# Newiz430/CellSegmentation

Measured on AMD Instinct MI355X. Metric: tiles/sec fwd+bwd (ResNet-50 MIL, 299x299), higher is better.
Workload: dtype bf16; 1 GPU; ResNet-50 tile classifier (train_tile.py --scratch semantics: fwd + CE + full bwd + Adam), bag=64 tiles of 299x299x3 per GPU, freeze_bn=True; tiles_per_gpu=64, parallelism=dp1

## Files before the change

cellsegmentation_amd/_lib.py:

```python
import ctypes
import os
from ctypes import POINTER, Structure, c_char_p, c_double, c_float, c_int, c_int32, c_int64, c_longlong, c_size_t, c_void_p

_HERE = os.path.dirname(os.path.abspath(__file__))
FLAVOUR = os.environ.get("CELLSEG_LIB_FLAVOUR", "")
if FLAVOUR not in ("", "ab"):
    raise RuntimeError(f"CELLSEG_LIB_FLAVOUR={FLAVOUR!r}: expected unset or 'ab'")
LIB_PATH = os.path.join(_HERE, f"libcellseg_hip_{FLAVOUR}.so" if FLAVOUR else "libcellseg_hip.so")

CS_F32, CS_BF16 = 0, 1
CS_ACT_NONE, CS_ACT_RELU, CS_ACT_SILU, CS_ACT_SIGMOID = 0, 1, 2, 3
CS_BN_BWD_OWN_RELU, CS_BN_BWD_FROZEN = 0x100, 0x200


class CsConvGeom(Structure):
    _fields_ = [(n, c_int32) for n in ("N", "H", "W", "C", "K", "R", "S", "stride", "pad", "P", "Q", "groups")]


class CsStageDesc(Structure):
    _fields_ = ([(n, c_void_p) for n in ("w", "gamma", "beta", "mean", "var", "conv_bias", "w_khwc", "w_chwk", "scale", "shift", "rstd")]
                + [("eps", c_float)] + [(n, c_int32) for n in ("K", "Cin", "R", "S", "Cp", "Kp", "block0", "fwd_packed", "bwd_packed")])


class CellsegLibraryMissing(RuntimeError):
# ... 50 lines not shown
    "cs_sgd_step_dev": (c_int, [_P, _P, c_int, c_int, _P, c_int, _P, c_double, c_double, c_int, c_int, _P]),
    "cs_sample_sum_workspace": (c_size_t, [c_int, c_int, c_int]),
    "cs_sample_sum": (c_int, [_P, _P, c_int, c_float, _P, _P, c_int, c_int, c_int, _P]),
    "cs_maxpool3x3s2_fwd": (c_int, [_P, c_int, _P, _P, c_int, c_int, c_int, c_int, c_int, c_int, _P]),
    "cs_maxpool3x3s2_bwd": (c_int, [_P, _P, _P, c_int, _P, c_int, c_int, c_int, c_int, c_int, c_int, _P]),
    "cs_gap_avgmax_fwd": (c_int, [_P, c_int, _P, _P, c_int, c_int, c_int, c_int, _P]),
    "cs_gap_avgmax_bwd": (c_int, [_P, _P, _P, c_int, _P, c_int, c_int, c_int, c_int, c_int, _P]),
    "cs_linear_fwd": (c_int, [_P, _P, _P, _P, _P, c_int, c_int, c_int, c_int, _P]),
    "cs_linear_bwd_workspace": (c_size_t, [c_int, c_int, c_int]),
    "cs_linear_bwd": (c_int, [_P, _P, _P, _P, c_int, _P, _P, _P, c_int, c_int, c_int, c_int, _P, _P]),
    "cs_loss_words": (c_int, []),
    "cs_softmax_ce": (c_int, [_P, _P, c_float, _P, _P, c_int, c_int, _P]),
    "cs_softmax_prob1": (c_int, [_P, _P, c_int, c_int, _P]),
    "cs_softmax_argmax": (c_int, [_P, _P, c_int, c_int, _P]),
    "cs_mse": (c_int, [_P, _P, c_int, c_int, _P, _P, c_int, _P]),
    "cs_bn_accum_words": (c_size_t, [c_int]),
    "cs_bn_accum_read": (c_int, [_P, c_int, _P, _P]),
    "cs_bn_stats": (c_int, [_P, c_int, c_longlong, c_int, _P, _P, _P]),
    "cs_bn_partial_workspace": (c_size_t, [c_longlong, c_int]),
    "cs_bn_finalize": (c_int, [_P, c_longlong, c_float, c_float, _P, _P, _P, _P, c_int, _P]),
    "cs_bn_apply": (c_int, [_P, c_int, _P, _P, _P, _P, _P, c_int, _P, c_longlong, c_int, _P]),
    "cs_bn_apply_stats": (c_int, [_P, c_int, _P, c_float, c_float, _P, _P, _P, _P, _P, c_int, _P, _P, _P, c_longlong, c_int, _P]),
    "cs_bn_bwd_reduce": (c_int, [_P, _P, c_int, _P, _P, _P, _P, c_int, c_longlong, c_int, _P, _P, _P]),
    "cs_bn_bwd_apply": (c_int, [_P, _P, c_int, _P, _P, _P, _P, c_int, _P, c_longlong, c_int, _P, _P, _P, _P]),
    "cs_dwconv_fwd": (c_int, [POINTER(CsConvGeom), c_int, _P, _P, _P, _P, c_int, _P, _P]),
    "cs_dwconv_fwd_stats_workspace": (c_size_t, [POINTER(CsConvGeom)]),
    "cs_dwconv_fwd_stats": (c_int, [POINTER(CsConvGeom), c_int, _P, _P, _P, _P, POINTER(c_int), _P]),
    "cs_bn_partial_fold": (c_int, [_P, c_int, c_int, _P, _P]),
    "cs_dwconv_dgrad": (c_int, [POINTER(CsConvGeom), c_int, _P, _P, _P, _P]),
    "cs_dwconv_wgrad": (c_int, [POINTER(CsConvGeom), c_int, _P, _P, _P, _P, _P]),
    "cs_dwconv_wgrad_oihw": (c_int, [POINTER(CsConvGeom), c_int, _P, _P, _P, _P, _P]),
    "cs_dw_weights_hwc_multi": (c_int, [_P, c_int, ctypes.c_longlong, _P]),
    "cs_dwconv_wgrad_workspace": (ctypes.c_size_t, [POINTER(CsConvGeom)]),
    "cs_se_scale": (c_int, [_P, c_int, _P, _P, c_int, c_int, c_int, _P]),
    "cs_se_scale_bwd_dx": (c_int, [_P, c_int, _P, _P, _P, c_int, c_int, c_int, _P]),
    "cs_rowscale_add": (c_int, [_P, c_int, _P, _P, _P, c_int, c_longlong, _P]),
    "cs_bilinear_ac_fwd": (c_int, [_P, c_int, _P, c_int, c_int, c_int, c_int, c_int, c_int, _P]),
    "cs_bilinear_ac_bwd": (c_int, [_P, _P, c_int, _P, c_int, c_int, c_int, c_int, c_int, c_int, _P]),
    "cs_concat_channels": (c_int, [_P, _P, c_int, _P, c_longlong, c_int, c_int, _P]),
    "cs_split_channels": (c_int, [_P, c_int, _P, _P, c_longlong, c_int, c_int, _P]),
    "cs_tile_gather": (c_int, [_P, c_int, c_int, c_int, _P, _P, c_longlong, c_int, POINTER(c_float), POINTER(c_float), c_int, _P, _P]),
    "cs_stage_augmented_workspace": (c_size_t, [c_longlong]),
    "cs_stage_augmented": (c_int, [_P, c_int, c_int, c_int, _P, _P, _P, _P, _P, c_int, c_longlong, c_int, c_int, POINTER(c_float),
                                   POINTER(c_float), c_int, _P, _P, c_size_t, _P]),
    "cs_dice_fwd": (c_int, [_P, _P, c_int, c_longlong, c_float, c_int, _P, _P, _P]),
    "cs_dice_bwd": (c_int, [_P, _P, _P, c_int, c_longlong, c_float, c_int, _P, _P]),
    "cs_softmax_channel_fwd": (c_int, [_P, _P, c_int, c_int, c_longlong, c_int, _P]),
    "cs_softmax_channel_bwd": (c_int, [_P, _P, _P, c_int, c_int, c_longlong, c_int, _P]),
    "cs_segmented_topk_workspace": (c_size_t, [c_longlong]),
    "cs_segmented_topk": (c_int, [_P, _P, _P, _P, c_int, c_int, c_longlong, _P, _P, _P, c_size_t, _P]),
    "cs_stem_pair_input": (c_int, [_P, c_int, c_int, c_int, c_int, _P, _P]),
    "cs_stem_pair_from_nchw": (c_int, [_P, c_int, c_int, c_int, c_int, _P, _P]),
    "cs_stem_fwd_packed": (c_int, [c_int, c_int, c_int, c_int, _P, _P, _P, c_int, _P, _P, _P]),
    "cs_stem_pair_weights": (c_int, [_P, c_int, c_int, _P, _P]),
    "cs_stem_fwd": (c_int, [c_int, c_int, c_int, c_int, c_int, _P, _P, _P, _P, c_int, _P, _P, _P, _P]),
    "cs_stem_wgrad_splits": (c_int, [c_int, c_int, c_int, c_int]),
    "cs_stem_wgrad": (c_int, [c_int, c_int, c_int, c_int, c_int, _P, _P, _P, c_int, _P]),
    "cs_stem_unpair_slabs": (c_int, [_P, c_int, c_int, _P, _P]),
    "cs_segmented_order": (c_int, [_P, _P, c_int, c_int, c_longlong, _P, _P]),
    "cs_threshold_select": (c_int, [_P, _P, c_longlong, c_float, _P, _P, _P, c_size_t, _P]),
    "cs_evaluate_tile_counts": (c_int, [_P, _P, _P, _P, c_float, c_longlong, _P, _P]),
    "cs_paint_tile_masks": (c_int, [_P, c_longlong, _P, _P, c_int, c_int, c_int, _P, _P]),
    "cs_prune_excess": (c_int, [_P, c_longlong, c_int, c_longlong, _P, _P, _P]),
    "cs_detect_quantize": (c_int, [_P, c_longlong, _P, _P]),
    "cs_detect_blur": (c_int, [_P, c_int, c_int, c_int, c_int, _P, c_int, _P, c_int, _P, _P]),
    "cs_stitch_workspace": (c_size_t, [c_int, c_int]),
    "cs_stitch_patches": (c_int, [_P, c_int, c_int, c_int, _P, c_int, c_int, _P, _P, c_size_t, _P]),
    "cs_stitch_logits": (c_int, [_P, c_int, c_int, c_int, c_int, c_int, _P, c_int, c_int, _P, _P]),
    "cs_detect_grid_size": (c_int, [c_int, c_int, c_int, c_int]),
    "cs_detect_meanshift": (c_int, [_P, c_int, c_int, c_int, c_int, c_int, c_double, c_int, _P, _P, _P]),
    "cs_detect_cluster_workspace": (c_size_t, [c_int, c_int]),
    "cs_detect_cluster": (c_int, [_P, _P, c_int, c_int, c_double, _P, c_int, c_int, c_int, _P, _P, _P, _P, c_size_t, _P]),
    "cs_detect_edt_workspace": (c_size_t, [c_int, c_int, c_int, c_int]),
    "cs_detect_edt_sq": (c_int, [_P, c_int, c_int, c_int, c_int, c_int, _P, _P, c_size_t, _P]),
    "cs_detect_edt_smooth": (c_int, [_P, c_int, c_int, c_int, c_int, c_int, _P, _P, c_size_t, _P]),
    "cs_morph_max_site_width": (c_int, []),
    "cs_morph_workspace": (c_size_t, [c_int, c_int, c_int]),
    "cs_morph_nearest": (c_int, [_P, c_int, c_int, c_int, c_int, c_int, _P, _P, _P, c_size_t, _P]),
    "cs_morph_binary": (c_int, [_P, c_int, c_int, c_int, c_int, c_int, c_int, _P, _P, c_size_t, _P]),
    "cs_morph_expand_labels": (c_int, [_P, c_int, c_int, c_int, c_int, _P, _P, c_size_t, _P]),
    "cs_regions_workspace": (c_size_t, [c_int, c_int, c_int]),
    "cs_regions_label": (c_int, [_P, c_int, c_int, c_int, c_int, _P, _P, c_size_t, _P]),
    "cs_regions_areas": (c_int, [_P, c_int, c_int, c_int, c_int, _P, _P, c_size_t, _P]),
    "cs_regions_filter": (c_int, [_P, c_int, c_int, c_int, c_int, c_int, c_int, _P, _P, c_size_t, _P]),
    "cs_regions_remove_small": (c_int, [_P, c_int, c_int, c_int, c_int, c_int, c_int, _P, _P, c_size_t, _P]),
    "cs_regions_threshold": (c_int, [_P, c_longlong, c_float, _P, _P]),
    "cs_regions_hsv_gate": (c_int, [_P, _P, c_longlong, c_int, _P, _P]),
    "cs_regions_number": (c_int, [_P, c_int, c_int, c_int, c_int, _P, _P, c_size_t, _P]),
    "cs_regions_measure": (c_int, [_P, _P, c_int, c_int, c_int, c_int, c_int, c_int, _P, _P, _P, _P, _P, _P, _P, c_size_t, _P]),
    "cs_regions_split_workspace": (c_size_t, [c_int, c_int, c_int, c_int]),
    "cs_regions_split": (c_int, [_P, c_int, c_int, c_int, c_int, _P, _P, _P, c_int, _P, _P, _P, _P, c_size_t, _P]),
    "cs_regions_geodesic_workspace": (c_size_t, [c_int, c_int, c_int, c_int]),
    "cs_regions_split_geodesic": (c_int, [_P, c_int, c_int, c_int, c_int, _P, _P, _P, c_int, c_int, c_int, _P, _P, _P, _P, _P, _P, c_size_t, _P]),
    "cs_regions_measure_labels": (c_int, [_P, _P, c_int, c_int, c_int, c_int, _P, _P, _P, _P, _P, _P, _P]),
    "cs_regions_edges_labels": (c_int, [_P, c_int, c_int, c_int, _P, _P]),
    "cs_regions_shape_labels": (c_int, [_P, _P, c_int, c_int, c_int, c_int, _P, _P, _P, _P]),
    "cs_regions_hull_max_side": (c_int, []),
    "cs_regions_hull_labels": (c_int, [_P, c_int, c_int, c_int, c_int, _P, _P, _P]),
    "cs_regions_match_workspace": (c_size_t, [c_int, c_int, c_int]),
    "cs_regions_match_labels": (c_int, [_P, _P, c_int, c_int, c_int, c_int, c_int, _P, _P, _P, _P, _P, _P, _P, _P, c_size_t, _P]),
    "cs_regions_overlap_workspace": (c_size_t, [c_int, c_int, c_int, c_int]),
    "cs_regions_overlap_labels": (c_int, [_P, _P] + [c_int] * 6 + [_P] * 13 + [c_size_t, _P]),
    "cs_regions_hausdorff_stage_runs": (c_int, []),
    "cs_regions_hausdorff_workspace": (c_size_t, [c_int, c_int, c_int]),
    "cs_regions_hausdorff_labels": (c_int, [_P, _P] + [c_int] * 5 + [_P] * 7 + [c_size_t, _P]),
    "cs_score_workspace": (c_size_t, [c_int, c_longlong]),
# ... 47 lines not shown
```

cellsegmentation_amd/engine.py:

```python
from collections import namedtuple
from types import SimpleNamespace

import torch

from . import _capture
from . import kernels as K

ACT_NONE, ACT_RELU, ACT_SILU = K.CS_ACT_NONE, K.CS_ACT_RELU, K.CS_ACT_SILU

PACKED = True
PACKED_TRAIN_BN = True


class ConvUnit:
    kind = "conv"

    def __init__(self, name, conv, bn, act, src, dst, res=None):
        self.name, self.conv, self.bn, self.act = name, conv, bn, act
        self.src, self.dst, self.res = src, dst, res
        self.grouped = conv.groups != 1
        if self.grouped:
            cg = conv.in_channels // conv.groups
            if conv.in_channels != conv.out_channels or conv.in_channels % 64 != 0 or 64 % cg != 0 or conv.bias is not None:
                raise NotImplementedError(f"{name}: grouped convolution needs C == K, C % 64 == 0, (C/groups) | 64, no bias "
                                          "(the ResNeXt 32x4d / 32x8d 3x3 layers)")
        self._cache = None

    def params(self):
        out = [("weight", self.conv.weight)]
        if self.conv.bias is not None:
            out.append(("bias", self.conv.bias))
        if self.bn is not None:
            out += [("gamma", self.bn.weight), ("beta", self.bn.bias)]
        return out

    def inputs(self):
        return [self.src] + ([self.res] if self.res is not None else [])

    def fwd(self, f, ui):
        x = f.t[self.src]
        N, H, W, Cp = x.shape
        conv = self.conv
        Kp = K.pad_channels(conv.out_channels)
        R, S = conv.kernel_size
        geom = K.make_geom(N, H, W, Cp, Kp, R, S, conv.stride[0], conv.padding[0])
        res = f.t[self.res] if self.res is not None else None
        batch_stats = _bn_uses_batch_stats(self.bn, f.bn_train)
        st = f.staged(ui, self, geom, batch_stats)
        stem = _is_paired_stem(self) and K.is_stem_geom(geom)
        xp = wp = None
        if ui == 0 and f.nchw_for_stem is not None:
            if not stem:
                raise RuntimeError("engine: the stem was expected to take the NCHW image (placeholder input would be read)")
            xp = K.stem_pair_from_nchw(f.nchw_for_stem, f.dtype)
        elif stem:
            xp = K.stem_pair_input(x)
        if stem:
            wp = K.stem_pair_weights(st.w_khwc)
        if batch_stats:
            stats = f.take_stats(Kp)
            if stem:
                z = K.stem_fwd(geom, xp, wp, None, st.shift, ACT_NONE, stats=stats)
            elif st.fwd_packed:
                z = K.conv_fwd_packed(geom, x, st.w_khwc, st.shift, None, ACT_NONE)
                K.bn_stats(z, stats)
            else:
                z = K.conv_fwd(geom, x, st.w_khwc, None, st.shift, None, ACT_NONE, stats=stats, grouped=self.grouped)
            y, mean, rstd = f.bn_train_fwd(self.bn, z, stats, res, self.act)
            f.aux[ui] = SimpleNamespace(geom=geom, st=st, train=True, z=z if f.save else None, mean=mean, rstd=rstd, xp=xp)
        else:
            want_bits = f.save and self.act == ACT_RELU
            if stem and PACKED and K.stem_fwd_packed_supported(geom, f.dtype):
                y = K.stem_fwd_packed(geom, xp, K.stem_pack_weights(wp), st.shift, self.act)
            elif stem:
                y = K.stem_fwd(geom, xp, wp, None, st.shift, self.act)
            elif st.fwd_packed and want_bits:
                y, f.bits[self.dst] = K.conv_fwd_packed(geom, x, st.w_khwc, st.shift, res, self.act, want_bits=True)
            elif st.fwd_packed:
                y = K.conv_fwd_packed(geom, x, st.w_khwc, st.shift, res, self.act)
            elif want_bits and Kp % 32 == 0:
                y, f.bits[self.dst] = K.conv_fwd(geom, x, st.w_khwc, None, st.shift, res, self.act, grouped=self.grouped, want_bits=True)
            else:
                y = K.conv_fwd(geom, x, st.w_khwc, None, st.shift, res, self.act, grouped=self.grouped)
            f.aux[ui] = SimpleNamespace(geom=geom, st=st, train=False, xp=xp)
        f.t[self.dst] = y

    def bwd(self, b, ui, g):
        a = b.aux[ui]
        x = b.t[self.src]
        if self.res is not None and b.requires.get(self.res, False):
            b.contribute(self.res, g, masked=False)
        if self.act == ACT_SILU and not a.train:
            raise NotImplementedError(f"{self.name}: backward through a folded (eval-mode) BN + SiLU is not supported; "
                                      "EfficientNet trains with batch statistics (efficientnet.py:308-312)")
        dz = b.bn_bwd(ui, self, g, a, self.conv.out_channels) if a.train else g
        if _defers(self, a, b.need, ui):
            b.defer_wgrad(ui, self, a, x, g, dz)
        elif b.need(ui, "weight") or b.need(ui, "bias") or (not a.train and (b.need(ui, "gamma") or b.need(ui, "beta"))):
            b.conv_wgrad(ui, self, a, x, g, dz)
        b.gsum_cache.pop(self.dst, None)
        if b.requires.get(self.src, False):
            b.grads[self.src] = b.conv_dgrad(self, a, x, dz)


class DwConvUnit:
    kind = "dw"

    def __init__(self, name, conv, bn, act, src, dst):
        self.name, self.conv, self.bn, self.act, self.src, self.dst = name, conv, bn, act, src, dst
        if conv.groups != conv.in_channels or conv.in_channels != conv.out_channels or conv.bias is not None:
            raise ValueError(f"{name}: not a bias-free depthwise convolution")

    def params(self):
        return [("weight", self.conv.weight), ("gamma", self.bn.weight), ("beta", self.bn.bias)]

    def inputs(self):
        return [self.src]

    def fwd(self, f, ui):
        x = f.t[self.src]
        N, H, W, C = x.shape
        conv, bn = self.conv, self.bn
        R = conv.kernel_size[0]
        geom = K.make_geom(N, H, W, C, C, R, R, conv.stride[0], conv.padding[0])
# ... 56 lines not shown
            b.emit(ui, "w2", dw2.view_as(self.fc2.weight))
        if b.need(ui, "b2"):
            b.emit(ui, "b2", db2)
        if b.need(ui, "w1"):
            b.emit(ui, "w1", dw1.view_as(self.fc1.weight))
        if b.need(ui, "b1"):
            b.emit(ui, "b1", db1)
        if b.requires.get(self.src, False):
            b.sole_consumer(self.src, "SE")
            b.grads[self.src] = K.se_scale_bwd_dx(g, a.s, davg)


class RowScaleAddUnit:
    kind = "sd"

    def __init__(self, a, b, dst, p):
        self.a, self.b, self.dst, self.p = a, b, dst, p

    def params(self):
        return []

    def inputs(self):
        return [self.a, self.b]

    def fwd(self, f, ui):
        a = f.t[self.a]
        keep = 1.0 - self.p
        noise = torch.empty((a.shape[0],), dtype=torch.float32, device=a.device).bernoulli_(keep)
        if keep > 0:
            noise.div_(keep)
        f.t[self.dst] = K.rowscale_add(a, noise, f.t[self.b])
        f.aux[ui] = SimpleNamespace(noise=noise)

    def bwd(self, b, ui, g):
        if b.requires.get(self.b, False):
            b.contribute(self.b, g, masked=True)
        if b.requires.get(self.a, False):
            b.contribute(self.a, K.rowscale_add(g, b.aux[ui].noise, None), masked=True)


class PoolUnit:
    kind = "pool"

    def __init__(self, src, dst):
        self.src, self.dst = src, dst

    def params(self):
        return []

    def inputs(self):
        return [self.src]

    def fwd(self, f, ui):
        x = f.t[self.src]
        f.t[self.dst], am = K.maxpool_fwd(x, want_argmax=f.save)
        f.aux[ui] = SimpleNamespace(argmax=am, in_hw=tuple(x.shape[1:3]))

    def bwd(self, b, ui, g):
        if b.requires.get(self.src, False):
            b.sole_consumer(self.src, "pool")
            a = b.aux[ui]
            b.grads[self.src] = K.maxpool_bwd(g, a.argmax, None, a.in_hw)


class UpsampleUnit:
    kind = "up"

    def __init__(self, src, dst, size_like=None, size_fn=None):
        self.src, self.dst, self.size_like, self.size_fn = src, dst, size_like, size_fn

    def params(self):
        return []

    def inputs(self):
        return [self.src]

    def fwd(self, f, ui):
        x = f.t[self.src]
        size = tuple(f.t[self.size_like].shape[1:3]) if self.size_like is not None else tuple(self.size_fn(f.in_hw))
        f.t[self.dst] = K.bilinear_fwd(x, size)
        f.aux[ui] = SimpleNamespace(in_hw=tuple(x.shape[1:3]))

    def bwd(self, b, ui, g):
        if b.requires.get(self.src, False):
            b.sole_consumer(self.src, "upsample")
            mask = b.t[self.src] if self.src in b.plan.relu_slots else None
            b.grads[self.src] = K.bilinear_bwd(g, b.aux[ui].in_hw, mask=mask)


class ConcatUnit:
    kind = "cat"

    def __init__(self, a, b, dst):
        self.a, self.b, self.dst = a, b, dst

    def params(self):
        return []

    def inputs(self):
        return [self.a, self.b]

    def fwd(self, f, ui):
        a, b = f.t[self.a], f.t[self.b]
        f.t[self.dst] = K.concat(a, b)
        f.aux[ui] = SimpleNamespace(ca=a.shape[-1])

    def bwd(self, b, ui, g):
        na, nb = b.requires.get(self.a, False), b.requires.get(self.b, False)
        if na or nb:
            ga, gb = K.split(g, b.aux[ui].ca, want_a=na, want_b=nb)
            if na:
                b.contribute(self.a, ga, masked=True)
            if nb:
                b.contribute(self.b, gb, masked=True)


class Plan:
    def __init__(self, units, inputs, outputs, relu_inputs=()):
        self.units, self.inputs, self.outputs = units, list(inputs), list(outputs)
        self.relu_slots = set(relu_inputs)
        for u in units:
            if u.kind == "conv" and u.act == ACT_RELU:
                self.relu_slots.add(u.dst)
            elif u.kind == "pool" and u.src in self.relu_slots:
                self.relu_slots.add(u.dst)
            elif u.kind == "cat" and u.a in self.relu_slots and u.b in self.relu_slots:
                self.relu_slots.add(u.dst)
        self.consumers = {}
        for u in units:
            for s in u.inputs():
                self.consumers[s] = self.consumers.get(s, 0) + 1
        self.param_list = []
        for ui, u in enumerate(units):
            for role, t in u.params():
                self.param_list.append((ui, role, t))

    def param_tensors(self):
        return [t for _, _, t in self.param_list]


def _bn_uses_batch_stats(bn, bn_train):
    return bn is not None and bn_train and bn.training


def _is_paired_stem(u):
    if u.kind != "conv":
        return False
    c = u.conv
    return (not u.grouped and u.res is None and c.in_channels <= 3 and c.kernel_size == (7, 7)
            and c.stride == (2, 2) and c.padding == (3, 3))


def _stem_takes_nchw(plan, dtype):
    if not (dtype == torch.bfloat16 and len(plan.inputs) == 1 and plan.units):
        return False
    u = plan.units[0]
    return (_is_paired_stem(u) and u.conv.in_channels == 3 and u.src == plan.inputs[0]
            and plan.consumers.get(u.src, 0) == 1)


def _packed_flags(plan, u, geom, dtype, need_bwd, batch_stats, bits, bn_train=False):
    if not PACKED or u.grouped or u.act not in (ACT_NONE, ACT_RELU):
        return False, False
    if batch_stats:
        if not (PACKED_TRAIN_BN and geom.R == 3 and geom.S == 3 and geom.stride == 1 and min(geom.C, geom.K) >= 128):
            return False, False
        pkf = K.packed_supported(geom, dtype, dgrad=False)
        pkb = bool(need_bwd) and K.packed_supported(geom, dtype, dgrad=True) and geom.C % 32 == 0
        return pkf, pkb
    pkf = K.packed_supported(geom, dtype, dgrad=False)
    pkb = bool(need_bwd) and K.packed_supported(geom, dtype, dgrad=True) and (u.src not in plan.relu_slots or u.src in bits)
    if pkb and geom.stride != 1:
        pkb = _compact_partner(plan, u, geom, dtype, bits, bn_train) is not None
    return pkf, pkb


def _compact_partner(plan, u, geom, dtype, bits, bn_train=False):
    others = [(i, v) for i, v in enumerate(plan.units) if v is not u and v.kind == "conv" and v.src == u.src]
    if len(others) != 1 or plan.consumers.get(u.src, 0) != 2:
        return None
    iv, v = others[0]
    iu = plan.units.index(u)
    c = v.conv
    if iv > iu or v.grouped or v.act not in (ACT_NONE, ACT_RELU) or c.kernel_size != (1, 1) or c.stride != (1, 1) or c.padding != (0, 0):
        return None
    if not PACKED or _bn_uses_batch_stats(v.bn, bn_train):
        return None
    if u.src in plan.relu_slots and u.src not in bits:
        return None
    gv = K.make_geom(geom.N, geom.H, geom.W, geom.C, K.pad_channels(c.out_channels), 1, 1, 1, 0)
    if not K.packed_supported(gv, dtype, dgrad=True):
        return None
    return v


_STAGE_EPOCH = [0]


def invalidate_staged():
    _STAGE_EPOCH[0] += 1


_StageSpec = namedtuple("_StageSpec", "Cp Kp need_bwd pkf pkb batch_stats")
# ... 429 lines not shown
```

cellsegmentation_amd/kernels.py:

```python
import ctypes

import torch

from . import _lib
from ._lib import (CS_ACT_NONE, CS_ACT_RELU, CS_ACT_SIGMOID, CS_ACT_SILU, CS_BF16, CS_BN_BWD_FROZEN, CS_BN_BWD_OWN_RELU, CS_F32,
                   CsConvGeom)


def _code(dtype):
    if dtype == torch.float32:
        return CS_F32
    if dtype == torch.bfloat16:
        return CS_BF16
    raise TypeError(f"unsupported activation dtype {dtype}; use torch.float32 or torch.bfloat16")


def _f32(*tensors):
    for t in tensors:
        if t.dtype != torch.float32:
            raise TypeError(f"this kernel reads torch.float32 only, got {t.dtype}; cast on the way in (functional.py does)")


def chunk(dtype):
    return 4 if dtype == torch.float32 else 8
# ... 286 lines not shown
    N, H, W, C = x.shape
    if C != 8:
        raise ValueError("stem_pair_input expects an NHWC image with 8 stored channels")
    out = torch.empty((N, H, (W + 1) // 2, 8), dtype=x.dtype, device=x.device)
    _lib.check(_lib.load().cs_stem_pair_input(_p(x), _code(x.dtype), N, H, W, _p(out), _stream()), "stem_pair_input")
    return out


def stem_pair_from_nchw(x_nchw, dtype):
    N, C, H, W = x_nchw.shape
    if C != 3 or x_nchw.dtype != torch.float32 or not x_nchw.is_contiguous():
        raise ValueError("stem_pair_from_nchw expects a contiguous fp32 [N,3,H,W] image")
    out = torch.empty((N, H, (W + 1) // 2, 8), dtype=dtype, device=x_nchw.device)
    _lib.check(_lib.load().cs_stem_pair_from_nchw(_p(x_nchw), _code(dtype), N, H, W, _p(out), _stream()), "stem_pair_from_nchw")
    return out


def stem_pair_weights(w_khwc):
    K_ = w_khwc.shape[0]
    out = torch.empty((K_, 7, 4, 8), dtype=w_khwc.dtype, device=w_khwc.device)
    _lib.check(_lib.load().cs_stem_pair_weights(_p(w_khwc), _code(w_khwc.dtype), K_, _p(out), _stream()), "stem_pair_weights")
    return out


def stem_fwd(geom, x_pair, w_pair, scale=None, shift=None, act=CS_ACT_NONE, stats=None):
    y = torch.empty((geom.N, geom.P, geom.Q, geom.K), dtype=x_pair.dtype, device=x_pair.device)
    lib = _lib.load()
    ws = _stats_ws(geom.N * geom.P * geom.Q, geom.K, x_pair.device) if stats is not None else None
    _lib.check(_timed("fwd", geom, x_pair.dtype, lambda: lib.cs_stem_fwd(
        geom.N, geom.H, geom.W, geom.K, _code(x_pair.dtype), _p(x_pair), _p(w_pair), _p(scale), _p(shift), act, _p(y), _p(stats), _p(ws),
        _stream())), "stem_fwd")
    return y


def stem_pack_weights(w_pair):
    K_ = w_pair.shape[0]
    w256 = torch.zeros((K_, 1, 1, 256), dtype=w_pair.dtype, device=w_pair.device)
    w256.view(K_, 256)[:, :224] = w_pair.reshape(K_, 224)
    return pack_conv_weights(make_geom(1, 2, 2, 256, K_, 1, 1, 1, 0), w256, dgrad=False)


def stem_fwd_packed_supported(geom, dtype):
    return dtype == torch.bfloat16 and is_stem_geom(geom) and geom.K == 64 and geom.P >= 2 and geom.Q >= 2


def stem_fwd_packed(geom, x_pair, w_packed, shift=None, act=CS_ACT_NONE, want_bits=False):
    y = torch.empty((geom.N, geom.P, geom.Q, geom.K), dtype=x_pair.dtype, device=x_pair.device)
    bits = torch.empty((geom.N, geom.P, geom.Q, geom.K // 8), dtype=torch.uint8, device=x_pair.device) if want_bits else None
    lib = _lib.load()
    _lib.check(_timed("fwd", geom, x_pair.dtype, lambda: lib.cs_stem_fwd_packed(
        geom.N, geom.H, geom.W, geom.K, _p(x_pair), _p(w_packed), _p(shift), act, _p(y), _p(bits), _stream()),
        extra_tensors=1.0 / 16 if want_bits else 0), "stem_fwd_packed")
    return (y, bits) if want_bits else y


def stem_wgrad(geom, x_pair, dy, use_tr_read=True):
    lib = _lib.load()
    nsplit = lib.cs_stem_wgrad_splits(geom.N, geom.H, geom.W, geom.K)
    pair = torch.empty((nsplit, geom.K, 7, 4, 8), dtype=torch.float32, device=dy.device)
    _lib.check(_timed("wgrad", geom, dy.dtype, lambda: lib.cs_stem_wgrad(
        geom.N, geom.H, geom.W, geom.K, _code(dy.dtype), _p(x_pair), _p(dy), _p(pair), 1 if use_tr_read else 0, _stream())), "stem_wgrad")
    raw = torch.empty((1, geom.K, 7, 7, 8), dtype=torch.float32, device=dy.device)
    _lib.check(lib.cs_stem_unpair_slabs(_p(pair), nsplit, geom.K, _p(raw), _stream()), "stem_unpair_slabs")
    return raw


class PartialColsum:

    def __init__(self, buf, rows, n_out):
        self.buf, self.rows, self.n_out = buf, rows, n_out
        self._vec = None
        self._vec_stream = None

    def _set(self, vec):
        self._vec, self._vec_stream = vec, torch.cuda.current_stream()

    def _sync(self):
        cur = torch.cuda.current_stream()
        if self._vec_stream is not None and cur != self._vec_stream:
            cur.wait_stream(self._vec_stream)
        return self._vec

    def vector(self):
        if self._vec is None:
            vec = torch.zeros((self.n_out,), dtype=torch.float32, device=self.buf.device)
            _lib.check(_lib.load().cs_fold_partial_rows(_p(self.buf), self.rows, self.n_out, _p(vec), _stream()), "fold_partial_rows")
            self._set(vec)
        return self._sync()


def colsum_vector(g):
    return g.vector() if isinstance(g, PartialColsum) else g


def conv_dgrad(geom, dy, w_chwk, add=None, mask=None, colsum=None, grouped=False, defer_colsum=False, mask_bits=None):
    dx = torch.empty((geom.N, geom.H, geom.W, geom.C), dtype=dy.dtype, device=dy.device)
    lib = _lib.load()
    geom = _grouped_geom(geom, grouped)
    defer = defer_colsum and not grouped and (geom.stride == 1 or lib.cs_conv2d_dgrad_partial_rows(ctypes.byref(geom)) > 0)
    ws = _stats_ws(geom.N * geom.H * geom.W, geom.C, dy.device) if (colsum is not None or defer) else None
    if mask_bits is not None:
        _lib.check(_timed("dgrad", geom, dy.dtype, lambda: lib.cs_conv2d_dgrad_bits(
            ctypes.byref(geom), _code(dy.dtype), _p(dy), _p(w_chwk), _p(add), _p(mask_bits), _p(dx), None if defer else _p(colsum), _p(ws),
            _stream()), extra_tensors=int(add is not None) + 1.0 / (8 * dx.element_size())), "conv2d_dgrad_bits")
    else:
        _lib.check(_timed("dgrad", geom, dy.dtype, lambda: lib.cs_conv2d_dgrad(
# ... 1201 lines not shown
```

include/cellseg_hip.h:

```cpp
#ifndef CELLSEG_HIP_H_
#define CELLSEG_HIP_H_

#include <stdint.h>
#include <stddef.h>

#ifdef __cplusplus
extern "C" {
#endif

enum { CS_F32 = 0, CS_BF16 = 1 };
enum { CS_OK = 0, CS_ERR_INVALID_ARG = -1, CS_ERR_LAUNCH = -2, CS_ERR_UNSUPPORTED = -3 };
enum { CS_ACT_NONE = 0, CS_ACT_RELU = 1, CS_ACT_SILU = 2, CS_ACT_SIGMOID = 3 };

int cs_abi_version(void);
const char* cs_last_error(void);
const char* cs_last_conv_variant(void);

typedef struct CsConvGeom {
    int32_t N, H, W, C;
    int32_t K;
    int32_t R, S;
    int32_t stride, pad;
    int32_t P, Q;
    int32_t groups;
// ... 128 lines not shown
                    void* stream);

int cs_tile_gather(const uint8_t* images, int n_images, int H, int W, const int32_t* tile_img, const int32_t* tile_rc,
                   long long n_tiles, int size, const float* host_mean3, const float* host_std3, int dtype, void* out,
                   void* stream);

size_t cs_stage_augmented_workspace(long long n_tiles);
int cs_stage_augmented(const uint8_t* images, int n_images, int H, int W, const int32_t* tile_img, const int32_t* tile_rc,
                       const int8_t* flips, const int8_t* jitter_ops, const float* jitter_factors, int has_contrast,
                       long long n_tiles, int th, int tw, const float* host_mean3, const float* host_std3, int dtype, void* out,
                       void* workspace, size_t workspace_bytes, void* stream);

int cs_linear_fwd(const float* x, const float* w, const float* b, float* y, float* preact, int M, int N, int K, int act,
                  void* stream);
size_t cs_linear_bwd_workspace(int M, int N, int K);
int cs_linear_bwd(const float* x, const float* w, const float* dy, const float* y, int act, float* dx, float* dw,
                  float* db, int M, int N, int K, int accumulate, float* workspace, void* stream);
int cs_loss_words(void);
int cs_softmax_ce(const float* logits, const int64_t* labels, float gamma, float* loss, float* dlogits, int M, int C,
                  void* stream);
int cs_softmax_prob1(const float* logits, float* p1, int M, int C, void* stream);
int cs_softmax_argmax(const float* logits, int64_t* idx, int M, int C, void* stream);
int cs_mse(const float* x, const float* t, int weighted, int mean, float* loss, float* dx, int M, void* stream);

int cs_dice_fwd(const float* p, const float* t, int N, long long HW, float eps, int mean, double* sums, float* loss,
                void* stream);
int cs_dice_bwd(const float* p, const float* t, const double* sums, int N, long long HW, float eps, int mean, float* dp,
                void* stream);
int cs_softmax_channel_fwd(const float* logits, float* pc, int N, int C, long long HW, int ch, void* stream);
int cs_softmax_channel_bwd(const float* logits, const float* dpc, float* dlogits, int N, int C, long long HW, int ch,
                           void* stream);

size_t cs_segmented_topk_workspace(long long T);
int cs_segmented_topk(const float* probs, const int32_t* groups, const int32_t* k_per_tile,
                      const int64_t* seg_offsets, int n_groups, int max_run, long long T, int64_t* out_idx,
                      int64_t* out_count, void* workspace, size_t workspace_bytes, void* stream);

int cs_conv2d_packed_supported(const CsConvGeom* g, int dgrad);
size_t cs_conv2d_packed_weight_bytes(const CsConvGeom* g, int dgrad);
int cs_pack_conv_weights(const CsConvGeom* g, int dgrad, const void* w_staged, void* w_packed, void* stream);
int cs_conv2d_packed_partial_rows(const CsConvGeom* g, int dgrad);
int cs_conv2d_fwd_packed(const CsConvGeom* g, const void* x, const void* w_packed, const float* shift, const void* residual, int act,
                         void* y, uint8_t* positive_bits, void* stream);
int cs_conv2d_dgrad_packed(const CsConvGeom* g, const void* dy, const void* w_packed, const void* add, int add_stride,
                           const uint8_t* mask_bits, void* dx, float* partial_rows, void* stream);

int cs_stem_pair_input(const void* x_nhwc8, int dtype, int N, int H, int W, void* x_pair, void* stream);
int cs_stem_pair_from_nchw(const float* x_nchw, int dtype, int N, int H, int W, void* x_pair, void* stream);
int cs_stem_pair_weights(const void* w_khwc, int dtype, int K, void* w_pair, void* stream);
int cs_stem_fwd(int N, int H, int W, int K, int dtype, const void* x_pair, const void* w_pair, const float* scale, const float* shift,
                int act, void* y, double* stats, void* workspace, void* stream);
int cs_stem_fwd_packed(int N, int H, int W, int K, const void* x_pair, const void* w_packed, const float* shift, int act, void* y,
                       uint8_t* positive_bits, void* stream);
int cs_stem_wgrad_splits(int N, int H, int W, int K);
int cs_stem_wgrad(int N, int H, int W, int K, int dtype, const void* x_pair, const void* dy, float* dw_pair_slabs, int use_tr_read,
                  void* stream);
int cs_stem_unpair_slabs(const float* dw_pair_slabs, int nsplit, int K, float* dw_khwc, void* stream);

int cs_segmented_order(const float* probs, const int64_t* seg_offsets, int n_groups, int max_run, long long T, int64_t* order,
                       void* stream);
int cs_threshold_select(const float* probs, const int64_t* order, long long T, float threshold, int64_t* out_idx,
                        int64_t* out_count, void* workspace, size_t workspace_bytes, void* stream);
int cs_evaluate_tile_counts(const float* probs, const int64_t* order, const int32_t* groups, const int64_t* pos_from,
                            float threshold, long long T, unsigned long long* counts4, void* stream);
int cs_paint_tile_masks(const int64_t* selected, long long n_selected, const int32_t* groups, const int32_t* tile_xy,
                        int tile_size, int H, int W, uint8_t* masks, void* stream);
int cs_prune_excess(const int32_t* labels, long long n, int flag, long long n_excess, int64_t* kept, int64_t* kept_count,
                    void* stream);

int cs_detect_quantize(const float* probs, long long n, uint8_t* out, void* stream);
int cs_detect_blur(const void* src, int src_is_f32, int N, int H, int W, const int32_t* taps_x, int kx, const int32_t* taps_y, int ky,
                   uint8_t* dst, void* stream);
size_t cs_stitch_workspace(int H, int W);
int cs_stitch_patches(const uint8_t* patches, int M, int ph, int pw, const int32_t* corners, int H, int W, uint8_t* out,
                      void* workspace, size_t workspace_bytes, void* stream);
int cs_stitch_logits(const float* logits, int B, int C, int ph, int pw, int ch, const int32_t* corners, int H, int W, uint8_t* mask,
                     void* stream);
int cs_detect_grid_size(int H, int W, int interval, int window);
int cs_detect_meanshift(const uint8_t* blurred, int N, int H, int W, int interval, int window, double thr255, int max_iter,
                        int32_t* pts, int32_t* n_pts, void* stream);
size_t cs_detect_cluster_workspace(int N, int cap);
int cs_detect_cluster(const int32_t* pts, const int32_t* n_pts, int N, int cap, double eps, const uint8_t* blurred, int H, int W,
                      int force_global, int64_t* out_pts, int32_t* out_w, int64_t* out_off, void* workspace,
                      size_t workspace_bytes, void* stream);
size_t cs_detect_edt_workspace(int N, int H, int W, int smooth);
int cs_detect_edt_sq(const void* src, int src_is_f32, int N, int H, int W, int thr, int32_t* d2, void* workspace,
                     size_t workspace_bytes, void* stream);
int cs_detect_edt_smooth(const void* src, int src_is_f32, int N, int H, int W, int thr, uint8_t* dst, void* workspace,
                         size_t workspace_bytes, void* stream);

int cs_morph_max_site_width(void);
size_t cs_morph_workspace(int N, int H, int W);
int cs_morph_nearest(const void* src, int src_is_labels, int background, int N, int H, int W, int32_t* d2, int32_t* site,
                     void* workspace, size_t workspace_bytes, void* stream);
int cs_morph_binary(const uint8_t* mask, int N, int H, int W, int erode, int r2, int outside_is_site, uint8_t* out, void* workspace,
                    size_t workspace_bytes, void* stream);
int cs_morph_expand_labels(const int32_t* labels, int N, int H, int W, int r2, int32_t* out, void* workspace, size_t workspace_bytes,
                           void* stream);

size_t cs_regions_workspace(int N, int H, int W);
int cs_regions_label(const uint8_t* mask, int N, int H, int W, int connectivity, int32_t* labels, void* workspace,
                     size_t workspace_bytes, void* stream);
int cs_regions_areas(const uint8_t* mask, int N, int H, int W, int connectivity, int32_t* areas, void* workspace,
                     size_t workspace_bytes, void* stream);
int cs_regions_filter(const uint8_t* mask, int N, int H, int W, int connectivity, int value, int min_area, uint8_t* out,
                      void* workspace, size_t workspace_bytes, void* stream);
// ... 72 lines not shown
```

Measured before the change: 9016 tiles/s.

## Fuse stem convolution, ReLU and 3x3 max-pool into one forward kernel

Adds a HIP kernel that computes the 7x7 stride-2 stem convolution with MFMA into an LDS tile, applies shift and ReLU, then runs the 3x3 stride-2 max-pool and writes the pooled output plus argmax indices directly. The engine routes the stem through this kernel when the pool is its only consumer, and the pool unit skips its own forward. This aims to avoid writing the full-resolution stem activation to HBM and reading it back for pooling. In exchange it recomputes halo rows and columns between tiles, and the stem output tensor is no longer materialised, which backward must not rely on.

```diff
diff --git a/cellsegmentation_amd/_lib.py b/cellsegmentation_amd/_lib.py
--- a/cellsegmentation_amd/_lib.py
+++ b/cellsegmentation_amd/_lib.py
@@ -126,6 +126,8 @@
     "cs_stem_pair_input": (c_int, [_P, c_int, c_int, c_int, c_int, _P, _P]),
     "cs_stem_pair_from_nchw": (c_int, [_P, c_int, c_int, c_int, c_int, _P, _P]),
     "cs_stem_fwd_packed": (c_int, [c_int, c_int, c_int, c_int, _P, _P, _P, c_int, _P, _P, _P]),
+    "cs_stem_pool_fwd_supported": (c_int, [c_int, c_int, c_int, c_int]),
+    "cs_stem_pool_fwd": (c_int, [c_int, c_int, c_int, c_int, _P, _P, _P, _P, _P, _P]),
     "cs_stem_pair_weights": (c_int, [_P, c_int, c_int, _P, _P]),
     "cs_stem_fwd": (c_int, [c_int, c_int, c_int, c_int, c_int, _P, _P, _P, _P, c_int, _P, _P, _P, _P]),
     "cs_stem_wgrad_splits": (c_int, [c_int, c_int, c_int, c_int]),
diff --git a/cellsegmentation_amd/csrc/stem_pool.hip b/cellsegmentation_amd/csrc/stem_pool.hip
--- /dev/null
+++ b/cellsegmentation_amd/csrc/stem_pool.hip
@@ -0,0 +1,254 @@
+#include <algorithm>
+#include "cs_common.h"
+
+namespace {
+
+#ifndef CS_STEM_POOL_TP
+#define CS_STEM_POOL_TP 5
+#define CS_STEM_POOL_TQ 15
+#endif
+
+struct SpParams {
+    const uint4* x;
+    const uint4* w;
+    const float* shift;
+    bf16_t* y;
+    uint8_t* amax;
+    int H, Wh, P, Q, PP, PQ;
+    unsigned N, tiles_x, tiles_y;
+};
+
+template <int TP, int TQ> struct SpTile {
+    static constexpr int SH = 2 * TP + 1, SW = 2 * TQ + 1;
+    static constexpr int NPIX = SH * SW, NT = (NPIX + 31) / 32;
+    static constexpr int NTW = (NT + 1) / 2;
+    static constexpr int WR = 4 * TP + 7, WP = 2 * TQ + 4;
+    static constexpr int NW = (WR * WP + 255) / 256;
+    static constexpr unsigned WIN_BYTES = (unsigned)NW * 4096u;
+    static constexpr unsigned ROW = 144u;
+    static constexpr unsigned TILE_BYTES = (unsigned)NPIX * ROW;
+    static constexpr unsigned LDS = WIN_BYTES + TILE_BYTES;
+    static_assert(LDS <= 81920u, "two workgroups per compute unit");
+    static_assert(6 * WP * 16 + 32 < 65536, "ds_read immediate offset");
+};
+
+__device__ __forceinline__ void swap_halves(unsigned& a, unsigned& b) {
+    auto r = __builtin_amdgcn_permlane32_swap(a, b, false, false);
+    a = r[0];
+    b = r[1];
+}
+
+template <int TP, int TQ>
+__global__ __launch_bounds__(256, 2) void stem_pool_fwd_kernel(SpParams p) {
+    using T = SpTile<TP, TQ>;
+    extern __shared__ __attribute__((aligned(16))) unsigned char smem[];
+    unsigned char* const win = smem;
+    unsigned char* const til = smem + T::WIN_BYTES;
+
+    const int tid = threadIdx.x, lane = tid & 63;
+    const int wave = __builtin_amdgcn_readfirstlane(tid >> 6);
+    const int l31 = lane & 31, hh = lane >> 5;
+    const int ct = wave & 1, tw = wave >> 1;
+
+    bf16x8 bw[14];
+#pragma unroll
+    for (int j = 0; j < 14; ++j) bw[j] = __builtin_bit_cast(bf16x8, p.w[(ct * 32 + l31) * 28 + 2 * j + hh]);
+    float sh[16];
+#pragma unroll
+    for (int g = 0; g < 4; ++g) {
+        float4 s4 = make_float4(0.f, 0.f, 0.f, 0.f);
+        if (p.shift) s4 = *reinterpret_cast<const float4*>(p.shift + ct * 32 + 8 * g + 4 * hh);
+        sh[4 * g] = s4.x; sh[4 * g + 1] = s4.y; sh[4 * g + 2] = s4.z; sh[4 * g + 3] = s4.w;
+    }
+    unsigned abase[T::NTW];
+#pragma unroll
+    for (int ti = 0; ti < T::NTW; ++ti) {
+        const int pi = (tw + 2 * ti) * 32 + l31;
+        const int pc = pi < T::NPIX ? pi : 0;
+        const int ly = pc / T::SW, lx = pc - ly * T::SW;
+        abase[ti] = (unsigned)((2 * ly * T::WP + lx + hh) * 16);
+    }
+
+    const unsigned n_tiles = p.tiles_x * p.tiles_y * p.N;
+    uint4 wv[T::NW];
+    unsigned wok = 0u;
+    auto fetch = [&](unsigned tile) {
+        const unsigned tx = tile % p.tiles_x, r1 = tile / p.tiles_x;
+        const unsigned ty = r1 % p.tiles_y;
+        const size_t n = r1 / p.tiles_y;
+        const int iy0 = 4 * (int)ty * TP - 5, px0 = 2 * (int)tx * TQ - 3;
+        const uint4* xi = p.x + n * (size_t)p.H * (size_t)p.Wh;
+        wok = 0u;
+#pragma unroll
+        for (int k = 0; k < T::NW; ++k) {
+            const int i = tid + 256 * k;
+            const int r = i / T::WP, c = i - r * T::WP;
+            const int iy = iy0 + r, px = px0 + c;
+            const bool ok = (unsigned)iy < (unsigned)p.H && (unsigned)px < (unsigned)p.Wh;
+            wv[k] = xi[ok ? (size_t)iy * (size_t)p.Wh + (size_t)px : (size_t)0];
+            wok |= ok ? 1u << k : 0u;
+        }
+    };
+    unsigned tile = blockIdx.x;
+    if (tile < n_tiles) fetch(tile);
+    for (; tile < n_tiles; tile += gridDim.x) {
+        const unsigned tx = tile % p.tiles_x, r1 = tile / p.tiles_x;
+        const unsigned ty = r1 % p.tiles_y;
+        const size_t n = r1 / p.tiles_y;
+        const int p0 = (int)ty * TP, q0 = (int)tx * TQ;
+#pragma unroll
+        for (int k = 0; k < T::NW; ++k)
+            reinterpret_cast<uint4*>(win)[tid + 256 * k] = (wok >> k) & 1u ? wv[k] : make_uint4(0u, 0u, 0u, 0u);
+        __syncthreads();
+        if (tile + gridDim.x < n_tiles) fetch(tile + gridDim.x);
+        __builtin_amdgcn_sched_barrier(0);
+
+        f32x16 acc[T::NTW];
+#pragma unroll
+        for (int ti = 0; ti < T::NTW; ++ti)
+#pragma unroll
+            for (int r = 0; r < 16; ++r) acc[ti][r] = 0.f;
+        bf16x8 af[2][T::NTW];
+#pragma unroll
+        for (int ti = 0; ti < T::NTW; ++ti) af[0][ti] = *reinterpret_cast<const bf16x8*>(win + abase[ti]);
+#pragma unroll
+        for (int j = 0; j < 14; ++j) {
+            const unsigned off = (unsigned)((((j + 1) >> 1) * T::WP + 2 * ((j + 1) & 1)) * 16);
+#pragma unroll
+            for (int ti = 0; ti < T::NTW; ++ti) {
+                if (j < 13) af[(j + 1) & 1][ti] = *reinterpret_cast<const bf16x8*>(win + abase[ti] + off);
+                acc[ti] = __builtin_amdgcn_mfma_f32_32x32x16_bf16(bw[j], af[j & 1][ti], acc[ti], 0, 0, 0);
+            }
+        }
+        __builtin_amdgcn_sched_group_barrier(0x100, T::NTW, 0);
+#pragma unroll
+        for (int k = 0; k < 13 * T::NTW; ++k) {
+            __builtin_amdgcn_sched_group_barrier(0x100, 1, 0);
+            __builtin_amdgcn_sched_group_barrier(0x008, 1, 0);
+        }
+        __builtin_amdgcn_sched_group_barrier(0x008, T::NTW, 0);
+#pragma unroll
+        for (int ti = 0; ti < T::NTW; ++ti) asm volatile("" : "+v"(acc[ti]));
+
+#pragma unroll
+        for (int ti = 0; ti < T::NTW; ++ti) {
+            if ((tw + 2 * ti) * 32 < T::NPIX) {
+                unsigned pk[8];
+#pragma unroll
+                for (int k = 0; k < 8; ++k) pk[k] = relu_bf16x2(pack_bf16x2(acc[ti][2 * k] + sh[2 * k], acc[ti][2 * k + 1] + sh[2 * k + 1]));
+                swap_halves(pk[0], pk[2]); swap_halves(pk[1], pk[3]);
+                swap_halves(pk[4], pk[6]); swap_halves(pk[5], pk[7]);
+                const int pi = (tw + 2 * ti) * 32 + l31;
+                if (pi < T::NPIX) {
+                    unsigned char* d = til + (unsigned)pi * T::ROW + (unsigned)((ct * 32 + 8 * hh) * 2);
+                    *reinterpret_cast<uint4*>(d) = make_uint4(pk[0], pk[1], pk[2], pk[3]);
+                    *reinterpret_cast<uint4*>(d + 32) = make_uint4(pk[4], pk[5], pk[6], pk[7]);
+                }
+            }
+        }
+        __syncthreads();
+
+        for (int i = tid; i < TP * TQ * 16; i += 256) {
+            const int c4 = i & 15, pq = i >> 4;
+            const int pp = pq / TQ, qq = pq - pp * TQ;
+            const int op = p0 + pp, oq = q0 + qq;
+            if (op >= p.PP || oq >= p.PQ) continue;
+            const unsigned char* w0 = til + (unsigned)(2 * pp * T::SW + 2 * qq) * T::ROW + (unsigned)c4 * 8u;
+            unsigned key[4] = {0u, 0u, 0u, 0u};
+    #pragma unroll
+            for (int t = 0; t < 9; ++t) {
+                const uint2 w = *reinterpret_cast<const uint2*>(w0 + (unsigned)((t / 3) * T::SW + t % 3) * T::ROW);
+                const unsigned c = 15u - (unsigned)t;
+                key[0] = max(key[0], (w.x << 16) | c);
+                key[1] = max(key[1], (w.x & 0xffff0000u) | c);
+                key[2] = max(key[2], (w.y << 16) | c);
+                key[3] = max(key[3], (w.y & 0xffff0000u) | c);
+            }
+            uint2 yv;
+            unsigned tv;
+            yv.x = (key[0] >> 16) | (key[1] & 0xffff0000u);
+            yv.y = (key[2] >> 16) | (key[3] & 0xffff0000u);
+            tv = 0x0f0f0f0fu - ((key[0] & 15u) | ((key[1] & 15u) << 8) | ((key[2] & 15u) << 16) | ((key[3] & 15u) << 24));
+            const bool inside = op > 0 && oq > 0 && 2 * op + 1 < p.P && 2 * oq + 1 < p.Q;
+            if (!inside || max(max(key[0], key[1]), max(key[2], key[3])) > 0x7f80ffffu) {
+                float best[4];
+                unsigned bi[4];
+    #pragma unroll
+                for (int e = 0; e < 4; ++e) { best[e] = -INFINITY; bi[e] = 0u; }
+                bool first = true;
+    #pragma unroll
+                for (int kh = 0; kh < 3; ++kh) {
+                    const int sy = 2 * op - 1 + kh;
+                    if (sy < 0 || sy >= p.P) continue;
+    #pragma unroll
+                    for (int kw = 0; kw < 3; ++kw) {
+                        const int sx = 2 * oq - 1 + kw;
+                        if (sx < 0 || sx >= p.Q) continue;
+                        const uint2 w = *reinterpret_cast<const uint2*>(w0 + (unsigned)(kh * T::SW + kw) * T::ROW);
+                        const float v[4] = {__uint_as_float(w.x << 16), __uint_as_float(w.x & 0xffff0000u), __uint_as_float(w.y << 16),
+                                            __uint_as_float(w.y & 0xffff0000u)};
+    #pragma unroll
+                        for (int e = 0; e < 4; ++e) {
+                            if (first || v[e] > best[e] || v[e] != v[e]) { best[e] = v[e]; bi[e] = (unsigned)(kh * 3 + kw); }
+                        }
+                        first = false;
+                    }
+                }
+                yv.x = pack_bf16x2(best[0], best[1]);
+                yv.y = pack_bf16x2(best[2], best[3]);
+                tv = bi[0] | (bi[1] << 8) | (bi[2] << 16) | (bi[3] << 24);
+            }
+            const size_t o = ((n * (size_t)p.PP + (size_t)op) * (size_t)p.PQ + (size_t)oq) * 64u + (size_t)c4 * 4u;
+            *reinterpret_cast<uint2*>(p.y + o) = yv;
+            if (p.amax) *reinterpret_cast<unsigned*>(p.amax + o) = tv;
+        }
+    }
+}
+
+struct SpShape {
+    int Wh, P, Q, PP, PQ;
+    unsigned tiles_x, tiles_y, grid;
+};
+bool sp_shape(int N, int H, int W, int K, SpShape& s) {
+    if (K != 64 || N <= 0 || H < 7 || W < 7) return false;
+    s.Wh = (W + 1) / 2;
+    s.P = (H - 1) / 2 + 1; s.Q = (W - 1) / 2 + 1;
+    s.PP = (s.P - 1) / 2 + 1; s.PQ = (s.Q - 1) / 2 + 1;
+    if ((long long)H * s.Wh * 16 >= (1ll << 31) || (long long)s.PP * s.PQ * 128 >= (1ll << 31)) return false;
+    s.tiles_x = (unsigned)cs_ceil_div(s.PQ, CS_STEM_POOL_TQ);
+    s.tiles_y = (unsigned)cs_ceil_div(s.PP, CS_STEM_POOL_TP);
+    const long long grid = (long long)N * s.tiles_x * s.tiles_y;
+    if (grid >= (1ll << 31)) return false;
+    s.grid = (unsigned)grid;
+    return true;
+}
+
+}
+
+extern "C" int cs_stem_pool_fwd_supported(int N, int H, int W, int K) {
+    SpShape s;
+    return sp_shape(N, H, W, K, s) ? 1 : 0;
+}
+
+extern "C" int cs_stem_pool_fwd(int N, int H, int W, int K, const void* x_pair, const void* w_pair, const float* shift, void* y_pool,
+                                uint8_t* argmax, void* stream) {
+    CS_CHECK_ARG(x_pair && w_pair && y_pool, "stem_pool_fwd: x_pair, w_pair and y_pool must not be NULL");
+    CS_CHECK_ARG(K == 64, "stem_pool_fwd: 64 output channels (the stem of every ResNet / ResNeXt of model/resnet.py)");
+    SpShape s;
+    CS_CHECK_ARG(sp_shape(N, H, W, K, s), "stem_pool_fwd: extents out of range (cs_stem_pool_fwd_supported)");
+    using T = SpTile<CS_STEM_POOL_TP, CS_STEM_POOL_TQ>;
+    auto fn = stem_pool_fwd_kernel<CS_STEM_POOL_TP, CS_STEM_POOL_TQ>;
+    SpParams p;
+    p.x = reinterpret_cast<const uint4*>(x_pair); p.w = reinterpret_cast<const uint4*>(w_pair); p.shift = shift;
+    p.y = reinterpret_cast<bf16_t*>(y_pool); p.amax = argmax;
+    p.H = H; p.Wh = s.Wh; p.P = s.P; p.Q = s.Q; p.PP = s.PP; p.PQ = s.PQ;
+    p.N = (unsigned)N; p.tiles_x = s.tiles_x; p.tiles_y = s.tiles_y;
+    if (!cs_allow_dynamic_lds_(reinterpret_cast<const void*>(fn), T::LDS, 81920)) return CS_ERR_LAUNCH;
+    char name[64];
+    snprintf(name, sizeof(name), "stem_pool_fwd_kernel<%d,%d>", CS_STEM_POOL_TP, CS_STEM_POOL_TQ);
+    cs_set_variant_(name);
+    const unsigned grid = std::min(s.grid, 2u * (unsigned)cs_device_cus_());
+    hipLaunchKernelGGL(fn, dim3(grid), dim3(256), T::LDS, reinterpret_cast<hipStream_t>(stream), p);
+    CS_LAUNCH_CHECK();
+    return CS_OK;
+}
diff --git a/cellsegmentation_amd/engine.py b/cellsegmentation_amd/engine.py
--- a/cellsegmentation_amd/engine.py
+++ b/cellsegmentation_amd/engine.py
@@ -10,6 +10,7 @@
 
 PACKED = True
 PACKED_TRAIN_BN = True
+FUSE_STEM_POOL = True
 
 
 class ConvUnit:
@@ -70,6 +71,14 @@
             f.aux[ui] = SimpleNamespace(geom=geom, st=st, train=True, z=z if f.save else None, mean=mean, rstd=rstd, xp=xp)
         else:
             want_bits = f.save and self.act == ACT_RELU
+            pool_ui = None
+            if stem and PACKED and FUSE_STEM_POOL and self.act == ACT_RELU and K.stem_pool_fwd_supported(geom, f.dtype):
+                pool_ui = _sole_pool_consumer(f.plan, self)
+            if pool_ui is not None:
+                f.t[f.plan.units[pool_ui].dst], am = K.stem_pool_fwd(geom, xp, wp, st.shift, want_argmax=f.save)
+                f.aux[pool_ui] = SimpleNamespace(argmax=am, in_hw=(geom.P, geom.Q))
+                f.aux[ui] = SimpleNamespace(geom=geom, st=st, train=False, xp=xp)
+                return
             if stem and PACKED and K.stem_fwd_packed_supported(geom, f.dtype):
                 y = K.stem_fwd_packed(geom, xp, K.stem_pack_weights(wp), st.shift, self.act)
             elif stem:
@@ -232,6 +241,8 @@
         return [self.src]
 
     def fwd(self, f, ui):
+        if f.aux[ui] is not None:
+            return
         x = f.t[self.src]
         f.t[self.dst], am = K.maxpool_fwd(x, want_argmax=f.save)
         f.aux[ui] = SimpleNamespace(argmax=am, in_hw=tuple(x.shape[1:3]))
@@ -329,6 +340,15 @@
     c = u.conv
     return (not u.grouped and u.res is None and c.in_channels <= 3 and c.kernel_size == (7, 7)
             and c.stride == (2, 2) and c.padding == (3, 3))
+
+
+def _sole_pool_consumer(plan, u):
+    if plan.consumers.get(u.dst, 0) != 1 or u.dst in plan.outputs:
+        return None
+    for vi, v in enumerate(plan.units):
+        if u.dst in v.inputs():
+            return vi if v.kind == "pool" else None
+    return None
 
 
 def _stem_takes_nchw(plan, dtype):
diff --git a/cellsegmentation_amd/kernels.py b/cellsegmentation_amd/kernels.py
--- a/cellsegmentation_amd/kernels.py
+++ b/cellsegmentation_amd/kernels.py
@@ -362,6 +362,21 @@
         geom.N, geom.H, geom.W, geom.K, _p(x_pair), _p(w_packed), _p(shift), act, _p(y), _p(bits), _stream()),
         extra_tensors=1.0 / 16 if want_bits else 0), "stem_fwd_packed")
     return (y, bits) if want_bits else y
+
+
+def stem_pool_fwd_supported(geom, dtype):
+    return (dtype == torch.bfloat16 and is_stem_geom(geom)
+            and bool(_lib.load().cs_stem_pool_fwd_supported(geom.N, geom.H, geom.W, geom.K)))
+
+
+def stem_pool_fwd(geom, x_pair, w_pair, shift, want_argmax=True):
+    PP, PQ = (geom.P - 1) // 2 + 1, (geom.Q - 1) // 2 + 1
+    y = torch.empty((geom.N, PP, PQ, geom.K), dtype=x_pair.dtype, device=x_pair.device)
+    am = torch.empty((geom.N, PP, PQ, geom.K), dtype=torch.uint8, device=x_pair.device) if want_argmax else None
+    lib = _lib.load()
+    _lib.check(_timed("fwd", geom, x_pair.dtype, lambda: lib.cs_stem_pool_fwd(
+        geom.N, geom.H, geom.W, geom.K, _p(x_pair), _p(w_pair), _p(shift), _p(y), _p(am), _stream())), "stem_pool_fwd")
+    return y, am
 
 
 def stem_wgrad(geom, x_pair, dy, use_tr_read=True):
diff --git a/include/cellseg_hip.h b/include/cellseg_hip.h
--- a/include/cellseg_hip.h
+++ b/include/cellseg_hip.h
@@ -204,6 +204,9 @@
                 int act, void* y, double* stats, void* workspace, void* stream);
 int cs_stem_fwd_packed(int N, int H, int W, int K, const void* x_pair, const void* w_packed, const float* shift, int act, void* y,
                        uint8_t* positive_bits, void* stream);
+int cs_stem_pool_fwd_supported(int N, int H, int W, int K);
+int cs_stem_pool_fwd(int N, int H, int W, int K, const void* x_pair, const void* w_pair, const float* shift, void* y_pool,
+                     uint8_t* argmax, void* stream);
 int cs_stem_wgrad_splits(int N, int H, int W, int K);
 int cs_stem_wgrad(int N, int H, int W, int K, int dtype, const void* x_pair, const void* dy, float* dw_pair_slabs, int use_tr_read,
                   void* stream);
```

Result: faster. 9134 tiles/s (median of 6 runs) (+1.3%).
